# ramosian-glider/syzkaller

Measured on AMD Instinct MI355X. Metric: coverage PCs triaged/sec vs corpus signal (+ % HBM roofline), 1/2/4/8 MI355X, higher is better.
Workload: dtype u32

## Files before the change

syzkaller_amd/csrc/sg_bucket.hip:

```cpp
#include "sg_internal.h"

#include <algorithm>

#ifndef SG_EXP
#define SG_EXP 0
#endif


namespace sg {

#ifndef SG_HT_ABL
#define SG_HT_ABL 0
#endif
#ifndef SG_PT
#define SG_PT 16384
#endif
#ifndef SG_PTHREADS
#define SG_PTHREADS 1024
#endif
constexpr int kPT = SG_PT;
constexpr int kPThreads = SG_PTHREADS;
constexpr int kPWaves = kPThreads / 64;
constexpr int kPerWave = kPT / kPWaves;
constexpr int kSteps = kPerWave / 64;
// ... 725 lines not shown
  const uint64_t* goff;
};

__device__ __forceinline__ uint32_t shard_of(uint32_t s, uint32_t nshards) {
  s ^= s >> 16;
  s *= 0x85EBCA6Bu;
  s ^= s >> 13;
  s *= 0xC2B2AE35u;
  s ^= s >> 16;
  return (uint32_t)(((uint64_t)s * nshards) >> 32);
}

constexpr uint32_t kMaxShards = 64;

template <int kPer>
__device__ __forceinline__ void emit_pairs(const BucketArgs& a, const uint32_t (&sig)[kPer], const uint32_t (&rec)[kPer],
                                           uint32_t* shcnt) {
  constexpr uint32_t kNone = 0xFFFFFFFFu;
  __shared__ uint32_t ewc[16];
  __shared__ unsigned long long ebase;
  const int lane = threadIdx.x & 63, w = threadIdx.x >> 6, nw = blockDim.x >> 6;
  uint32_t c = 0;
#pragma unroll
  for (int k = 0; k < kPer; k++) c += rec[k] != kNone ? 1u : 0u;
  uint32_t incl = c;
#pragma unroll
  for (int o = 1; o < 64; o <<= 1) {
    const uint32_t y = __shfl_up(incl, o);
    if (lane >= o) incl += y;
  }
  if (lane == 63) ewc[w] = incl;
  __syncthreads();
  if (threadIdx.x == 0) {
    uint32_t acc = 0;
    for (int i = 0; i < nw; i++) {
      const uint32_t v = ewc[i];
      ewc[i] = acc;
      acc += v;
    }
    ebase = acc ? atomicAdd(a.npairs, (unsigned long long)acc) : 0ull;
  }
  __syncthreads();
  uint64_t pos = ebase + ewc[w] + incl - c;
#pragma unroll
  for (int k = 0; k < kPer; k++)
    if (rec[k] != kNone) {
      a.pairs[pos++] = make_uint2(sig[k], a.rec_base + rec[k]);
      if (a.shard_cnt) atomicAdd(&shcnt[shard_of(sig[k], a.nshards)], 1u);
    }
  __syncthreads();
}

template <int kPer>
__device__ __forceinline__ void emit_grouped(const BucketArgs& a, const uint32_t (&sig)[kPer], const uint32_t (&rec)[kPer],
                                             uint32_t* lcnt, unsigned long long* lbase) {
  constexpr uint32_t kNone = 0xFFFFFFFFu;
#pragma unroll
  for (int k = 0; k < kPer; k++)
    if (rec[k] != kNone) atomicAdd(&lcnt[rec[k] >> kGroupBits], 1u);
  __syncthreads();
  for (uint32_t g = threadIdx.x; g < a.NG; g += blockDim.x) {
    const uint32_t c = lcnt[g];
    lbase[g] = c ? a.goff[(uint64_t)g << kGroupBits] + atomicAdd(&a.gcur[g], (unsigned long long)c) : 0ull;
    lcnt[g] = 0;
  }
  __syncthreads();
#pragma unroll
  for (int k = 0; k < kPer; k++)
    if (rec[k] != kNone) {
      const uint32_t g = rec[k] >> kGroupBits;
      a.pairs[lbase[g] + atomicAdd(&lcnt[g], 1u)] = make_uint2(sig[k], rec[k]);
    }
  __syncthreads();
  for (uint32_t g = threadIdx.x; g < a.NG; g += blockDim.x) lcnt[g] = 0;
  __syncthreads();
}

__device__ __forceinline__ void flush_shard_counts(const BucketArgs& a, const uint32_t* shcnt) {
  if (a.shard_cnt)
    for (uint32_t i = threadIdx.x; i < a.nshards; i += blockDim.x)
      if (shcnt[i]) atomicAdd(&a.shard_cnt[i], (unsigned long long)shcnt[i]);
}

__global__ void k_bucket_compact(const uint4* __restrict__ bdesc, const uint32_t* __restrict__ lpos,
                                 uint32_t* __restrict__ blist_b, uint4* __restrict__ blist_q) {
  const uint32_t b = blockIdx.x * blockDim.x + threadIdx.x;
  if (b >= kNumBuckets) return;
  const uint4 q = bdesc[b];
  if (q.x < q.y) {
    blist_b[lpos[b]] = b;
    blist_q[lpos[b]] = q;
  }
}

__global__ void k_bucket_desc(const uint32_t* __restrict__ goff2, const uint32_t* __restrict__ gcount,
                              const uint32_t* __restrict__ cfirst, uint4* __restrict__ bdesc, uint32_t* __restrict__ nz) {
  const uint32_t b = blockIdx.x * blockDim.x + threadIdx.x;
  if (b >= kNumBuckets) return;
  const uint32_t d = b >> 8, f = b & 255, c0 = cfirst[d], nch = cfirst[d + 1] - c0;
  const uint32_t* row = goff2 + (uint64_t)f * *gcount + c0;
  const uint32_t lo = row[0], hi = row[nch];
  bdesc[b] = make_uint4(lo, hi, c0, nch);
  nz[b] = lo < hi ? 1u : 0u;
}

__global__ void k_bucket_groups(const uint32_t* __restrict__ goff2, const uint32_t* __restrict__ gcount,
                                const uint32_t* __restrict__ cbase, uint32_t NG, uint32_t* __restrict__ gbnd) {
  const uint64_t i = (uint64_t)blockIdx.x * blockDim.x + threadIdx.x;
  if (i >= (uint64_t)kNumBuckets * NG) return;
  const uint32_t b = (uint32_t)(i / NG), g = (uint32_t)(i % NG);
  gbnd[i] = goff2[(uint64_t)(b & 255) * *gcount + cbase[(b >> 8) * NG + g]];
}

__device__ __forceinline__ uint32_t group_of(const uint32_t* gb, uint32_t NG, uint32_t p) {
  uint32_t lo = 0, hi = NG;
  while (hi - lo > 1) {
    const uint32_t mid = (lo + hi) >> 1;
    if (gb[mid] <= p)
      lo = mid;
    else
      hi = mid;
  }
  return lo;
}

__device__ __forceinline__ uint32_t entry_record(uint32_t g, uint32_t x) { return (g << kGroupBits) | (x & 0xFFFFu); }

constexpr uint32_t kGroupWords = (kMaxGroups + kBThreads - 1) / kBThreads;
constexpr int kWPT = kBucketWords / kBThreads;
typedef uint32_t wvec __attribute__((ext_vector_type(kWPT)));
struct BucketPre {
  uint32_t msw[kBucketWords / kBThreads];
  uint32_t nsw[kBucketWords / kBThreads];
  uint32_t gw[kGroupWords];
};

__device__ __forceinline__ uint32_t round_pos(uint32_t base, int u) { return base + threadIdx.x * kBU + u; }

__device__ __forceinline__ void bucket_round_load(const BucketArgs& a, uint32_t base, uint32_t hi,
                                                  uint32_t (&x)[kBU]) {
  const uint4* p = reinterpret_cast<const uint4*>(a.in + base) + threadIdx.x * (kBU / 4);
#pragma unroll
  for (int j = 0; j < kBU / 4; j++) {
    uint4 v = make_uint4(0, 0, 0, 0);
    if (round_pos(base, 4 * j) < hi) {
      const v4u32 t = __builtin_nontemporal_load(reinterpret_cast<const v4u32*>(p + j));
      v = make_uint4(t[0], t[1], t[2], t[3]);
    }
    x[4 * j] = v.x;
    x[4 * j + 1] = v.y;
    x[4 * j + 2] = v.z;
    x[4 * j + 3] = v.w;
  }
}

__device__ __forceinline__ void bucket_pre_load(const BucketArgs& a, uint32_t b, BucketPre& P) {
  const uint64_t w0 = bucket_word(b, kWPT * threadIdx.x);
  wvec m = *reinterpret_cast<const wvec*>(a.mwords + w0);
  if (a.owords) m |= *reinterpret_cast<const wvec*>(a.owords + w0);
  wvec nw = {};
  if (a.nwords) nw = *reinterpret_cast<const wvec*>(a.nwords + w0);
#pragma unroll
  for (int j = 0; j < kWPT; j++) {
    P.msw[j] = m[j];
    P.nsw[j] = nw[j];
  }
  const uint32_t* gr = a.gbnd + (uint64_t)b * a.NG;
#pragma unroll
  for (int j = 0; j < (int)kGroupWords; j++) {
    const uint32_t i = j * kBThreads + threadIdx.x;
    P.gw[j] = i < a.NG ? gr[i] : 0u;
  }
}

__device__ __forceinline__ uint32_t list_bucket(const BucketArgs& a, uint32_t t, uint32_t nl, uint4* q) {
  if (t >= nl) return kNumBuckets;
  *q = a.blist_q[t];
  return a.blist_b[t];
}

#ifndef SG_LDS_BARRIER
#define SG_LDS_BARRIER 0
#endif
__device__ __forceinline__ void lds_barrier() {
#if SG_LDS_BARRIER
  asm volatile("s_waitcnt lgkmcnt(0)\n\ts_barrier" ::: "memory");
#else
  __syncthreads();
#endif
}

__device__ __forceinline__ uint32_t uni(uint32_t v) { return __builtin_amdgcn_readfirstlane(v); }
__device__ __forceinline__ uint4 uni(uint4 v) { return make_uint4(uni(v.x), uni(v.y), uni(v.z), uni(v.w)); }

constexpr uint32_t kMapMul = 0x6F4Bu;
constexpr uint32_t inv16(uint32_t c) {
  uint32_t x = c;
  for (int i = 0; i < 4; i++) x = (x * (2u - c * x)) & 0xFFFFu;
  return x;
}
constexpr uint32_t kMapInv = inv16(kMapMul);
static_assert(((kMapMul * kMapInv) & 0xFFFFu) == 1u, "kMapInv");
static_assert(kHash == 8192 && kMaxProbe <= 31, "13-bit slots, 5-bit displacements");
static_assert((uint64_t)kMaxGroups << kGroupBits <= (1u << 24), "records fit 24 bits");
constexpr uint32_t kRecMask = 0xFFFFFFu;

__device__ __forceinline__ uint32_t map_signal(uint32_t slot, uint32_t v) {
  const uint32_t home = (slot - ((v >> 24) & 31u)) & (kHash - 1);
  return (((home << 3) | (v >> 29)) * kMapInv) & 0xFFFFu;
}

__device__ __forceinline__ bool map_insert(uint32_t* ht, uint32_t sl, uint32_t rec, uint32_t disp0 = 0) {
  const uint32_t y = (sl * kMapMul) & 0xFFFFu;
  const uint32_t home = y >> 3, tag = y & 7u;
  for (uint32_t disp = disp0; disp < kMaxProbe; disp++) {
    const uint32_t mine = (tag << 29) | (disp << 24) | rec;
    uint32_t* slot = &ht[(home + disp) & (kHash - 1)];
    const uint32_t old = atomicCAS(slot, kEmpty, mine);
    if (old == kEmpty) return true;
    if ((old >> 24) == (mine >> 24)) {
      if ((old & kRecMask) > rec) atomicMin(slot, mine);
      return true;
    }
  }
  return false;
}

__device__ __forceinline__ uint32_t take_ticket(uint32_t* p) { return atomicAdd(p, 1u); }
__device__ __forceinline__ void take_wait(uint32_t&) {}

template <bool kDbg, int kEmit>
__global__ __launch_bounds__(kBThreads) __attribute__((amdgpu_waves_per_eu(kBWaves))) void k_bucket(BucketArgs a) {
  __shared__ uint32_t mslice[kBucketWords];
  __shared__ uint32_t nbits[kBucketWords];
  __shared__ uint32_t ht[kHash];
  __shared__ alignas(16) uint32_t gb[kMaxGroups];
  __shared__ uint32_t sh_fail;
  __shared__ uint32_t sh_b[2];
  __shared__ uint4 sh_q[2];
  __shared__ uint32_t shcnt[kEmit == 1 ? kMaxShards : 1];
  __shared__ uint32_t lcnt[kEmit == 2 ? kMaxGroups : 1];
  __shared__ unsigned long long lbase[kEmit == 2 ? kMaxGroups : 1];
  const int tid = threadIdx.x;
  if (kEmit == 1)
    for (uint32_t i = tid; i < kMaxShards; i += kBThreads) shcnt[i] = 0;
  if (kEmit == 2)
    for (uint32_t i = tid; i < kMaxGroups; i += kBThreads) lcnt[i] = 0;
  const uint32_t NG = a.NG;
  constexpr uint32_t kRound = kBThreads * kBU;
  const uint64_t t_start = kDbg ? wall_clock64() : 0;
  uint64_t n_buckets = 0, n_rounds = 0;
  uint64_t ph[7] = {0, 0, 0, 0, 0, 0, 0};
  uint64_t tk = kDbg ? clock64() : 0;
  for (uint32_t i = tid; i < kHash; i += kBThreads) ht[i] = kEmpty;
  for (uint32_t i = tid; i < kBucketWords; i += kBThreads) nbits[i] = 0;
  if (tid == 0) sh_fail = 0;
  const uint32_t nl = *a.nlist;
  uint32_t pend_t = 0;
  if (tid == 0) {
    uint4 q0 = make_uint4(0, 0, 0, 0), q1 = make_uint4(0, 0, 0, 0);
    sh_b[0] = list_bucket(a, blockIdx.x, nl, &q0);
    sh_q[0] = q0;
    sh_b[1] = list_bucket(a, gridDim.x + blockIdx.x, nl, &q1);
    sh_q[1] = q1;
    pend_t = take_ticket(a.ticket);
  }
  __syncthreads();
  uint32_t b = uni(sh_b[0]), b1 = uni(sh_b[1]);
  uint4 q = uni(sh_q[0]), q1 = uni(sh_q[1]);
  if (b >= kNumBuckets) {
    if (tid == 0) take_wait(pend_t);
    if (kDbg && tid == 0) {
      for (int j = 0; j < 8; j++) a.dbg[8 * blockIdx.x + j] = 0;
      a.dbg[8 * blockIdx.x] = t_start;
      a.dbg[8 * blockIdx.x + 1] = wall_clock64();
    }
    return;
  }
  uint32_t x[kBU], y[kBU];
  BucketPre P;
  bucket_round_load(a, q.x & ~3u, q.y, x);
  bucket_pre_load(a, b, P);
  while (b < kNumBuckets) {
    const uint32_t lo = q.x, hi = q.y;
    lds_barrier();
    {
      wvec mv;
#pragma unroll
      for (int j = 0; j < kWPT; j++) mv[j] = P.msw[j];
      reinterpret_cast<wvec*>(mslice)[tid] = mv;
    }
    uint32_t ns[kWPT];
#pragma unroll
    for (int j = 0; j < kWPT; j++) ns[j] = P.nsw[j];
#pragma unroll
    for (int j = 0; j < (int)kGroupWords; j++) {
      const uint32_t i = j * kBThreads + tid;
      if (i < kMaxGroups) gb[i] = i < NG ? P.gw[j] : kEmpty;
    }
    uint32_t pend_b = kNumBuckets;
    uint4 pend_q = make_uint4(0, 0, 0, 0);
    if (tid == 0) {
      take_wait(pend_t);
      pend_b = list_bucket(a, 2 * gridDim.x + pend_t, nl, &pend_q);
      pend_t = take_ticket(a.ticket);
      if (kEmit) take_wait(pend_t);
      sh_fail = 0;
    }
    lds_barrier();
    const uint32_t gbl = NG <= 64 ? gb[threadIdx.x & 63] : kEmpty;
    if (kDbg) {
      const uint64_t t = clock64();
      ph[0] += t - tk;
      tk = t;
    }
    n_buckets++;
    for (uint32_t base = lo & ~3u;;) {
      n_rounds++;
      const uint32_t next = base + kRound;
      const bool last = next >= hi;
      if (!last || b1 < kNumBuckets) bucket_round_load(a, last ? q1.x & ~3u : next, last ? q1.y : hi, y);
      if (last && b1 < kNumBuckets) bucket_pre_load(a, b1, P);
      const uint32_t p0 = round_pos(base, 0);
      const uint32_t failed = __hip_atomic_load(&sh_fail, __ATOMIC_RELAXED, __HIP_MEMORY_SCOPE_WORKGROUP);
      uint32_t mw[kBU];
#pragma unroll
      for (int u = 0; u < kBU; u++) mw[u] = mslice[x[u] >> 21];
      uint32_t cm = 0;
#pragma unroll
      for (int u = 0; u < kBU; u++) {
        const uint32_t i = p0 + u;
        const uint32_t miss = ((~mw[u]) >> ((x[u] >> 16) & 31)) & 1u;
        cm |= (miss & (i >= lo ? 1u : 0u) & (i < hi ? 1u : 0u)) << u;
      }
      if (kDbg) {
        asm volatile("s_waitcnt lgkmcnt(0)" ::: "memory");
        const uint64_t t = clock64();
        ph[4] += t - tk;
        tk = t;
      }
      uint32_t gu[kBU];
      if (NG <= 64) {
        const uint32_t pw = base + (threadIdx.x & ~63u) * kBU;
        const uint32_t nle = (uint32_t)__popcll(__ballot(gbl <= pw));
#pragma unroll
        for (int u = 0; u < kBU; u++) gu[u] = nle;
// ... 157 lines not shown
      }
      __syncthreads();
      uint64_t pos = ebase + ewc[w] + incl - c;
      if (c) {
#pragma unroll
        for (int k = 0; k < kOwn; k++) {
          const uint32_t i = k * kBThreads + tid;
          const uint32_t v = ht[i];
          if (v != kEmpty) {
            const uint32_t sl = map_signal(i, v);
            const uint32_t sg = part_sig((b << 16) | sl);
            a.pairs[pos++] = make_uint2(sg, a.rec_base + (v & kRecMask));
            if (a.shard_cnt) atomicAdd(&shcnt[shard_of(sg, a.nshards)], 1u);
            if (a.nwords || a.update) atomicOr(&nbits[sl >> 5], 1u << (sl & 31));
            ht[i] = kEmpty;
          }
        }
      }
      __syncthreads();
      if (a.update) {
        const wvec nb = reinterpret_cast<const wvec*>(nbits)[tid];
        const wvec mw = reinterpret_cast<const wvec*>(mslice)[tid];
        const uint64_t w0 = bucket_word(b, kWPT * tid);
#pragma unroll
        for (int j = 0; j < kWPT; j++)
          if (nb[j]) {
            a.mwords[w0 + j] = mw[j] | nb[j];
            if (a.nwords) a.nwords[w0 + j] = ns[j] | nb[j];
          }
      } else if (a.nwords) {
        const wvec nb = reinterpret_cast<const wvec*>(nbits)[tid];
        uint32_t* ng = a.nwords + bucket_word(b, kWPT * tid);
#pragma unroll
        for (int j = 0; j < kWPT; j++)
          if (nb[j]) ng[j] = ns[j] | nb[j];
      }
      reinterpret_cast<wvec*>(nbits)[tid] = wvec{};
    } else {
      constexpr int kOwn = kHash / kBThreads;
      {
#pragma unroll
        for (int k = 0; k < kOwn; k++) {
          const uint32_t i = k * kBThreads + tid;
          const uint32_t v = ht[i];
          ht[i] = kEmpty;
          if (v != kEmpty) {
            const uint32_t sl = map_signal(i, v);
            atomicOr(&nbits[sl >> 5], 1u << (sl & 31));
            a.rec_new[v & kRecMask] = 1;
          }
        }
        lds_barrier();
      }
      {
        const uint64_t w0 = bucket_word(b, kWPT * tid);
        uint32_t* mg = a.mwords + w0;
        uint32_t* ng = a.nwords ? a.nwords + w0 : nullptr;
        const wvec nb = reinterpret_cast<const wvec*>(nbits)[tid];
        uint32_t any = 0;
#pragma unroll
        for (int j = 0; j < kWPT; j++) any |= nb[j];
        if (any) {
          const wvec mw = reinterpret_cast<const wvec*>(mslice)[tid];
#pragma unroll
          for (int j = 0; j < kWPT; j++)
            if (nb[j]) {
              mg[j] = mw[j] | nb[j];
              if (ng) ng[j] = ns[j] | nb[j];
            }
          reinterpret_cast<wvec*>(nbits)[tid] = wvec{};
        }
      }
    }
    if (kDbg) {
      const uint64_t t = clock64();
      ph[3] += t - tk;
      tk = t;
    }
    lds_barrier();
    if (kDbg) {
      const uint64_t t = clock64();
      ph[6] += t - tk;
      tk = t;
    }
    b = b1;
    q = q1;
    b1 = uni(sh_b[0]);
    q1 = uni(sh_q[0]);
#pragma unroll
    for (int u = 0; u < kBU; u++) x[u] = y[u];
  }
  if (kEmit == 1) {
    __syncthreads();
    flush_shard_counts(a, shcnt);
  }
  if (kDbg && tid == 0) {
    a.dbg[8 * blockIdx.x] = t_start;
    a.dbg[8 * blockIdx.x + 1] = wall_clock64();
    a.dbg[8 * blockIdx.x + 2] = n_buckets;
    a.dbg[8 * blockIdx.x + 3] = n_rounds;
    for (int j = 0; j < 4; j++) a.dbg[8 * blockIdx.x + 4 + j] = ph[j];
    a.dbg[8 * gridDim.x + 3 * blockIdx.x] = ph[4];
    a.dbg[8 * gridDim.x + 3 * blockIdx.x + 1] = ph[5];
    a.dbg[8 * gridDim.x + 3 * blockIdx.x + 2] = ph[6];
  }
}

constexpr int kDThreads = 1024;
template <bool kEmit>
__global__ __launch_bounds__(kDThreads) void k_bucket_direct(BucketArgs a) {
  constexpr uint32_t kQ = 8192, kNQ = 65536 / kQ, kQW = kQ / 32;
  __shared__ uint32_t owner[kQ];
  __shared__ uint32_t mpart[kQW];
  __shared__ uint32_t nbits[kQW];
  __shared__ uint32_t gb[kMaxGroups];
  __shared__ uint32_t shcnt[kEmit ? kMaxShards : 1];
  __shared__ uint32_t lcnt[kEmit ? kMaxGroups : 1];
  __shared__ unsigned long long lbase[kEmit ? kMaxGroups : 1];
  const int tid = threadIdx.x;
  const uint32_t nsp = *a.nspill, NG = a.NG;
  if (kEmit) {
    for (uint32_t i = tid; i < kMaxShards; i += kDThreads) shcnt[i] = 0;
    for (uint32_t i = tid; i < kMaxGroups; i += kDThreads) lcnt[i] = 0;
    __syncthreads();
  }
  for (uint32_t job = blockIdx.x; job < nsp * kNQ; job += gridDim.x) {
    const uint32_t b = a.spill[job / kNQ], qq = job % kNQ;
    const uint4 q = a.bdesc[b];
    for (uint32_t i = tid; i < kQW; i += kDThreads) {
      const uint64_t w = bucket_word(b, qq * kQW + i);
      mpart[i] = a.mwords[w] | (a.owords ? a.owords[w] : 0u);
      nbits[i] = 0;
    }
    for (uint32_t i = tid; i < NG; i += kDThreads) gb[i] = a.gbnd[(uint64_t)b * NG + i];
    for (uint32_t i = tid; i < kQ; i += kDThreads) owner[i] = kEmpty;
    __syncthreads();
    for (uint32_t i = q.x + tid; i < q.y; i += kDThreads) {
      const uint32_t x = a.in[i];
      const uint32_t sl = x >> 16, sq = sl % kQ;
      if (sl / kQ != qq || ((mpart[sq >> 5] >> (sq & 31)) & 1u)) continue;
      atomicMin(&owner[sq], entry_record(group_of(gb, NG, i), x));
      atomicOr(&nbits[sq >> 5], 1u << (sq & 31));
    }
    __syncthreads();
    if (kEmit) {
      constexpr int kPer = kQ / kDThreads;
      uint32_t sig[kPer], rec[kPer];
#pragma unroll
      for (int k = 0; k < kPer; k++) {
        const uint32_t i = k * kDThreads + tid;
        sig[k] = part_sig((b << 16) | (qq * kQ + i));
        rec[k] = owner[i];
      }
      if (a.gcur)
        emit_grouped(a, sig, rec, lcnt, lbase);
      else
        emit_pairs(a, sig, rec, shcnt);
      for (uint32_t i = tid; i < kQW; i += kDThreads) {
        const uint32_t nb = nbits[i];
        if (!nb) continue;
        const uint64_t w = bucket_word(b, qq * kQW + i);
        if (a.update) a.mwords[w] = mpart[i] | nb;
        if (a.nwords) a.nwords[w] |= nb;
      }
    } else {
      for (uint32_t i = tid; i < kQ; i += kDThreads)
        if (owner[i] != kEmpty) a.rec_new[owner[i]] = 1;
      for (uint32_t i = tid; i < kQW; i += kDThreads) {
        const uint32_t nb = nbits[i];
        if (nb) {
          const uint64_t w = bucket_word(b, qq * kQW + i);
          a.mwords[w] = mpart[i] | nb;
          if (a.nwords) a.nwords[w] |= nb;
        }
      }
    }
    __syncthreads();
  }
  if (kEmit) flush_shard_counts(a, shcnt);
}

constexpr int kScanThreads = 1024;
constexpr int kScanPer = 16;
constexpr uint32_t kScanTile = kScanThreads * kScanPer;

__device__ __forceinline__ uint32_t block_excl_scan(uint32_t v, uint32_t* wsum, uint32_t* total) {
  const int tid = threadIdx.x, lane = tid & 63, w = tid >> 6;
// ... 52 lines not shown
  __shared__ uint32_t wsum[16];
  __shared__ uint32_t tot;
  uint32_t carry = 0;
  for (uint64_t b0 = 0; b0 < nb; b0 += kScanThreads) {
    const uint64_t i = b0 + threadIdx.x;
    const uint32_t v = i < nb ? sums[i] : 0u;
    const uint32_t ex = block_excl_scan(v, wsum, &tot);
    if (i < nb) sums[i] = carry + ex;
    carry += tot;
    __syncthreads();
  }
}

__global__ __launch_bounds__(kScanThreads) void k_scan32_apply(const uint32_t* __restrict__ in, uint64_t n,
                                                               const uint32_t* __restrict__ n_dev, uint32_t mul,
                                                               const uint32_t* __restrict__ sums,
                                                               uint32_t* __restrict__ out) {
  __shared__ uint32_t wsum[16];
  __shared__ uint32_t tot;
  n = scan_n(n, n_dev, mul);
  const uint64_t b_last = n ? (n - 1) / kScanTile : 0;
  if (blockIdx.x > b_last) return;
  const uint64_t base = (uint64_t)blockIdx.x * kScanTile + (uint64_t)threadIdx.x * kScanPer;
  const bool full = base + kScanPer <= n;
  uint32_t v[kScanPer];
  uint32_t s = 0;
  if (full) {
#pragma unroll
    for (int k = 0; k < kScanPer; k += 4) {
      const uint4 q = *reinterpret_cast<const uint4*>(in + base + k);
      v[k] = q.x;
      v[k + 1] = q.y;
      v[k + 2] = q.z;
      v[k + 3] = q.w;
    }
  } else {
#pragma unroll
    for (int k = 0; k < kScanPer; k++) v[k] = base + k < n ? in[base + k] : 0u;
  }
#pragma unroll
  for (int k = 0; k < kScanPer; k++) s += v[k];
  uint32_t run = (sums ? sums[blockIdx.x] : 0u) + block_excl_scan(s, wsum, &tot);
  uint32_t o[kScanPer];
#pragma unroll
  for (int k = 0; k < kScanPer; k++) {
    o[k] = run;
    run += v[k];
  }
  if (full) {
#pragma unroll
    for (int k = 0; k < kScanPer; k += 4)
      *reinterpret_cast<uint4*>(out + base + k) = make_uint4(o[k], o[k + 1], o[k + 2], o[k + 3]);
  } else {
#pragma unroll
    for (int k = 0; k < kScanPer; k++)
      if (base + k < n) out[base + k] = o[k];
  }
  if (blockIdx.x == b_last && threadIdx.x == kScanThreads - 1) out[n] = run;
}

static size_t scan32_ws(uint64_t n) { return (((n + kScanTile - 1) / kScanTile) * 4 + 255) & ~size_t(255); }

static int scan32(sg_ctx* ctx, const uint32_t* in, uint32_t* out, uint64_t n, uint32_t* scratch,
                  const uint32_t* n_dev = nullptr, uint32_t mul = 1) {
  ScopedTimer tm(ctx, "scan");
  const uint64_t nb = (n + kScanTile - 1) / kScanTile;
  if (nb == 0) {
    SG_HIP(hipMemsetAsync(out, 0, 4, ctx->stream));
    return SG_OK;
  }
  if (nb == 1) {
    hipLaunchKernelGGL(k_scan32_apply, dim3(1), dim3(kScanThreads), 0, ctx->stream, in, n, n_dev, mul,
                       (const uint32_t*)nullptr, out);
    SG_HIP(hipGetLastError());
    return SG_OK;
  }
  hipLaunchKernelGGL(k_scan32_reduce, dim3((uint32_t)nb), dim3(kScanThreads), 0, ctx->stream, in, n, n_dev, mul,
                     scratch);
  hipLaunchKernelGGL(k_scan32_top, dim3(1), dim3(kScanThreads), 0, ctx->stream, scratch, nb);
  hipLaunchKernelGGL(k_scan32_apply, dim3((uint32_t)nb), dim3(kScanThreads), 0, ctx->stream, in, n, n_dev, mul,
                     scratch, out);
  SG_HIP(hipGetLastError());
  return SG_OK;
}

constexpr uint32_t kFRemBits = 11;
constexpr uint32_t kFBuckets = 1u << (24 - kFRemBits);
constexpr uint32_t kFOvBlocks = 1984;
constexpr uint32_t kFPad = 0x8000u;
constexpr uint32_t kFSpill = 512;
constexpr uint32_t kFHMax = 4;
constexpr uint32_t kFIdx = 256 * kFHMax;
constexpr uint32_t kFSurvCap = 1u << 20;
constexpr uint32_t kFTableBits = 21;
constexpr int kFThreads = 1024;
#ifndef SG_FPARTS
#define SG_FPARTS 8
#endif
#ifndef SG_FU
#define SG_FU 4
#endif
#ifndef SG_FEH
#define SG_FEH 4
#endif
#ifndef SG_FABL
#define SG_FABL 0
#endif
constexpr uint32_t kFParts = SG_FPARTS;
constexpr uint32_t kFWgCap = 4 * kFSurvCap / (256 * kFParts);
constexpr unsigned long long kFEmpty = ~0ull;

struct M0F {
  uint4* tab;
  uint16_t* ovals;
  uint32_t* cursor;
  uint32_t* nspill;
  uint32_t* spill;
  uint32_t* nsurv;
  uint2* surv;
  uint32_t* wgcnt;
  unsigned long long* table;
};
static size_t m0f_bytes() {
  return (uint64_t)kFIdx * kFBuckets * 16 + (uint64_t)kFIdx * kFOvBlocks * 16 + kFIdx * 4 + 256 + kFIdx * 4 +
         (uint64_t)kFIdx * kFSpill * 4 + 256ull * kFParts * kFWgCap * 8 +
         256ull * kFParts * 4 + (8ull << kFTableBits);
}
static M0F m0f_bind(sg_ctx* ctx) {
  char* b = (char*)ctx->m0f;
  M0F f;
  f.tab = (uint4*)b;
  b += (uint64_t)kFIdx * kFBuckets * 16;
  f.ovals = (uint16_t*)b;
  b += (uint64_t)kFIdx * kFOvBlocks * 16;
  f.cursor = (uint32_t*)b;
  f.nsurv = f.cursor + kFIdx;
  f.nspill = f.cursor + kFIdx + 64;
  b += kFIdx * 4 + 256 + kFIdx * 4;
  f.spill = (uint32_t*)b;
  b += (uint64_t)kFIdx * kFSpill * 4;
  f.surv = (uint2*)b;
  b += 256ull * kFParts * kFWgCap * 8;
  f.wgcnt = (uint32_t*)b;
  b += 256ull * kFParts * 4;
  f.table = (unsigned long long*)b;
  return f;
}

template <int kLogH>
__global__ __launch_bounds__(256) void k_m0_index(const uint32_t* __restrict__ mwords, uint4* __restrict__ tab,
                                                   uint16_t* __restrict__ ovals, uint32_t* __restrict__ cursor,
                                                   uint32_t* __restrict__ nspill, uint32_t* __restrict__ spill,
                                                   uint32_t* __restrict__ flags) {
  constexpr int kQ = 16 >> kLogH;
  constexpr uint32_t kRB = kFRemBits - kLogH;
  const uint32_t dh = blockIdx.y, lane = threadIdx.x & 63;
  const uint32_t d = dh >> kLogH, h = dh & ((1u << kLogH) - 1);
  const uint32_t j = blockIdx.x * 256 + threadIdx.x;
  const uint4* src = reinterpret_cast<const uint4*>(mwords + ((uint64_t)d << 19) + ((uint64_t)h << (19 - kLogH)) +
                                                    (uint64_t)j * (4 * kQ));
  uint4 q[kQ];
#pragma unroll
  for (int i = 0; i < kQ; i++) q[i] = src[i];
  uint32_t n = 0;
#pragma unroll
  for (int i = 0; i < kQ; i++) n += __popc(q[i].x) + __popc(q[i].y) + __popc(q[i].z) + __popc(q[i].w);
// ... 401 lines not shown
  uint32_t* v2 = (uint32_t*)ws_at(ctx, bp.oV2);
    uint32_t* scr = (uint32_t*)ws_at(ctx, bp.oSC);
  const uint32_t T = (uint32_t)bp.T, G = (uint32_t)bp.gmax, NG = (uint32_t)bp.NG;
  const uint32_t* gcount = cbase + bp.ng;
  const bool dbg = ctx->debug_part;
  if (stages & 1) {
  Cuts c1{};
  c1.nA = bp.nA;
  c1.step = kPT;
  c1.nB = bp.nB;
  c1.n = n;
  c1.rec_off = d_off;
  c1.nrec = nrec;
  c1.start = tstart;
  c1.aux = trec;
  hipLaunchKernelGGL(k_cuts, dim3(div_up(bp.T + 1, 256)), dim3(256), 0, ctx->stream, c1);
  hipLaunchKernelGGL(k_group_tiles, dim3(div_up(bp.NG + 1, 256)), dim3(256), 0, ctx->stream, d_off, bp.nA, NG, T,
                     gt);
  {
    ScopedTimer tm(ctx, "p1_hist");
    if (trace)
      hipLaunchKernelGGL(k_hist_trace, dim3(T), dim3(kPThreads), 0, ctx->stream, d_vals, d_off, nrec,
                         (const uint32_t*)tstart, (const uint32_t*)trec, T, hist1, (uint64_t*)ws_at(ctx, bp.oKM));
    else if (((uintptr_t)d_vals & 15) == 0)
      hipLaunchKernelGGL(k_hist_rep<false>, dim3(T), dim3(kPThreads), 0, ctx->stream, d_vals,
                         (const uint32_t*)tstart, (const uint4*)nullptr, T, (const uint32_t*)nullptr, hist1);
    else
      hipLaunchKernelGGL(k_p1_hist, dim3(T), dim3(kPThreads), 0, ctx->stream, d_vals,
                         (const uint32_t*)tstart, hist1);
  }
  rc = scan32(ctx, hist1, goff1, 256 * bp.T, scr);
  if (rc) return rc;
  P1Args a1{d_vals, d_off, nrec, tstart, trec, T, goff1, hist1, v1, plane ? b1 : nullptr, nullptr,
            (const uint64_t*)ws_at(ctx, bp.oKM)};
  unsigned long long* p1dbg = nullptr;
  if (dbg) {
    SG_HIP(hipMalloc(&p1dbg, 64));
    SG_HIP(hipMemsetAsync(p1dbg, 0, 64, ctx->stream));
    a1.dbg = p1dbg;
  }
  {
    ScopedTimer tm(ctx, "p1_scatter");
    if (dbg && trace)
      hipLaunchKernelGGL((k_p1_scatter<true, true>), dim3(T), dim3(kPThreads), 0, ctx->stream, a1);
    else if (dbg)
      hipLaunchKernelGGL((k_p1_scatter<true, false>), dim3(T), dim3(kPThreads), 0, ctx->stream, a1);
    else if (trace)
      hipLaunchKernelGGL((k_p1_scatter<false, true>), dim3(T), dim3(kPThreads), 0, ctx->stream, a1);
    else
      hipLaunchKernelGGL((k_p1_scatter<false, false>), dim3(T), dim3(kPThreads), 0, ctx->stream, a1);
  }
  if (dbg) {
    unsigned long long h[8];
    SG_HIP(hipMemcpy(h, p1dbg, 64, hipMemcpyDeviceToHost));
    SG_HIP(hipFree(p1dbg));
    fprintf(stderr, "sg p1_scatter per tile (cycles, wave 0): load+meta %.0f build+lookup %.0f rank %.0f stage %.0f "
            "write %.0f (tiles %llu)\n", (double)h[0] / h[5], (double)h[1] / h[5], (double)h[2] / h[5],
            (double)h[3] / h[5], (double)h[4] / h[5], h[5]);
  }
  }
  if (!(stages & 2)) return SG_OK;
  hipLaunchKernelGGL(k_group_chunks, dim3(div_up(bp.ng, 256)), dim3(256), 0, ctx->stream, (const uint32_t*)goff1,
                     T, NG, (const uint32_t*)gt, bp.ng, nch);
  rc = scan32(ctx, nch, cbase, bp.ng, scr);
  if (rc) return rc;
  hipLaunchKernelGGL(k_chunk_list, dim3(div_up((bp.ng > bp.gmax ? bp.ng : bp.gmax) + 1, 256)), dim3(256), 0,
                     ctx->stream, (const uint32_t*)goff1, T, NG, (const uint32_t*)gt, bp.ng,
                     (const uint32_t*)cbase, bp.gmax, cstart, cgov, cfirst);
  hipLaunchKernelGGL(k_chunk_desc, dim3(div_up(bp.gmax, 256)), dim3(256), 0, ctx->stream, (const uint32_t*)cstart,
                     (const uint32_t*)cgov, gcount, bp.gmax, (const uint32_t*)goff1, T, NG, (const uint32_t*)gt,
                     cdesc, dtile);
  {
    ScopedTimer tm(ctx, "p2_hist");
    hipLaunchKernelGGL(k_hist_bytes, dim3(G), dim3(kHBThreads), 0, ctx->stream, (const uint8_t*)b1,
                       (const uint4*)cdesc, gcount, hist2);
  }
  rc = scan32(ctx, hist2, goff2, 256 * bp.gmax, scr, gcount, 256);
  if (rc) return rc;
  P2Args a2{v1, cdesc, dtile, gcount, goff1, trec, T, NG, goff2, hist2, v2};
  {
    ScopedTimer tm(ctx, "p2_scatter");
    hipLaunchKernelGGL(k_p2_scatter, dim3(G), dim3(kPThreads), 0, ctx->stream, a2);
  }
  uint32_t* bnz = (uint32_t*)ws_at(ctx, bp.oBN);
  uint32_t* blpos = (uint32_t*)ws_at(ctx, bp.oBP);
  hipLaunchKernelGGL(k_bucket_desc, dim3(kNumBuckets / 256), dim3(256), 0, ctx->stream, (const uint32_t*)goff2,
                     gcount, (const uint32_t*)cfirst, bdesc, bnz);
  hipLaunchKernelGGL(k_bucket_groups, dim3(div_up((uint64_t)kNumBuckets * NG, 256)), dim3(256), 0, ctx->stream,
                     (const uint32_t*)goff2, gcount, (const uint32_t*)cbase, NG, gbnd);
  rc = scan32(ctx, bnz, blpos, kNumBuckets, scr);
  if (rc) return rc;
  hipLaunchKernelGGL(k_bucket_compact, dim3(kNumBuckets / 256), dim3(256), 0, ctx->stream, (const uint4*)bdesc,
                     (const uint32_t*)blpos, (uint32_t*)ws_at(ctx, bp.oLB), (uint4*)ws_at(ctx, bp.oLQ));
  SG_HIP(hipGetLastError());
  return SG_OK;
}

static int buckets_one(sg_ctx* ctx, const BucketPlan& bp, uint32_t* mwords, uint32_t* nwords, uint8_t* d_rec_new,
                       const EmitArgs* emit, uint64_t n, uint64_t nrec, const uint32_t* owords = nullptr) {
  const uint32_t NG = (uint32_t)bp.NG;
  const uint32_t* cbase = (const uint32_t*)ws_at(ctx, bp.oCB);
  const uint32_t* gcount = cbase + bp.ng;
  uint4* bdesc = (uint4*)ws_at(ctx, bp.oBD);
  uint32_t* gbnd = (uint32_t*)ws_at(ctx, bp.oGB);
  uint32_t* v2 = (uint32_t*)ws_at(ctx, bp.oV2);
  uint32_t* nspill = (uint32_t*)ws_at(ctx, bp.oSP);
  uint32_t* blpos = (uint32_t*)ws_at(ctx, bp.oBP);
  const bool dbg = ctx->debug_part;
  BucketArgs ba{};
  ba.in = v2;
  ba.bdesc = bdesc;
  ba.gbnd = gbnd;
  ba.NG = NG;
  ba.mwords = mwords;
  ba.owords = owords;
  ba.nwords = nwords;
  ba.rec_new = d_rec_new;
  ba.nspill = nspill;
  ba.spill = nspill + 1;
  ba.ticket = (uint32_t*)ws_at(ctx, bp.oTK);
  if (emit) {
    ba.pairs = emit->pairs;
    ba.npairs = emit->npairs;
    ba.rec_base = emit->rec_base;
    ba.nshards = emit->nshards;
    ba.shard_cnt = emit->shard_cnt;
    ba.update = emit->update ? 1u : 0u;
    ba.gcur = emit->gcur;
    ba.goff = emit->goff;
  }
  uint32_t bgrid = persistent_grid(ctx, (const void*)k_bucket<false, 0>, kBThreads);
  const int64_t cap_blocks = ctx->opt[kOptBucketBlocks];
  if (cap_blocks > 0 && (uint64_t)cap_blocks < bgrid) bgrid = (uint32_t)cap_blocks;
  uint64_t* ddbg = nullptr;
  if (dbg) {
    SG_HIP(hipMalloc(&ddbg, (size_t)bgrid * 88));
    ba.dbg = ddbg;
  }
  SG_HIP(hipMemsetAsync(ba.ticket, 0, 4, ctx->stream));
  SG_HIP(hipMemsetAsync(nspill, 0, 4, ctx->stream));
  ba.blist_b = (const uint32_t*)ws_at(ctx, bp.oLB);
  ba.blist_q = (const uint4*)ws_at(ctx, bp.oLQ);
  ba.nlist = blpos + kNumBuckets;
  {
    ScopedTimer tm(ctx, "bucket_triage");
    if (emit && emit->gcur)
      hipLaunchKernelGGL((k_bucket<false, 2>), dim3(bgrid), dim3(kBThreads), 0, ctx->stream, ba);
    else if (emit)
      hipLaunchKernelGGL((k_bucket<false, 1>), dim3(bgrid), dim3(kBThreads), 0, ctx->stream, ba);
    else if (dbg)
      hipLaunchKernelGGL((k_bucket<true, 0>), dim3(bgrid), dim3(kBThreads), 0, ctx->stream, ba);
    else
      hipLaunchKernelGGL((k_bucket<false, 0>), dim3(bgrid), dim3(kBThreads), 0, ctx->stream, ba);
  }
  {
    ScopedTimer tm(ctx, "bucket_spill");
    if (emit)
      hipLaunchKernelGGL(k_bucket_direct<true>, dim3(512), dim3(kDThreads), 0, ctx->stream, ba);
    else
      hipLaunchKernelGGL(k_bucket_direct<false>, dim3(512), dim3(kDThreads), 0, ctx->stream, ba);
  }
  SG_HIP(hipGetLastError());
  if (dbg) {
    uint32_t g = 0, sp = 0;
    SG_HIP(hipMemcpyAsync(&g, gcount, 4, hipMemcpyDeviceToHost, ctx->stream));
    SG_HIP(hipMemcpyAsync(&sp, nspill, 4, hipMemcpyDeviceToHost, ctx->stream));
    SG_HIP(hipStreamSynchronize(ctx->stream));
    fprintf(stderr, "sg part: n=%llu nrec=%llu tiles=%llu chunks=%u (bound %llu) spilled_buckets=%u\n",
            (unsigned long long)n, (unsigned long long)nrec, (unsigned long long)bp.T, g,
            (unsigned long long)bp.gmax, sp);
    std::vector<uint4> bd(kNumBuckets);
    std::vector<uint64_t> hd((size_t)bgrid * 11);
    SG_HIP(hipMemcpy(bd.data(), bdesc, bd.size() * 16, hipMemcpyDeviceToHost));
    SG_HIP(hipMemcpy(hd.data(), ddbg, hd.size() * 8, hipMemcpyDeviceToHost));
    double qa = 0, qb = 0, qc = 0;
    for (uint32_t i = 0; i < bgrid; i++) {
      qa += hd[8 * bgrid + 3 * i];
      qb += hd[8 * bgrid + 3 * i + 1];
      qc += hd[8 * bgrid + 3 * i + 2];
    }
    SG_HIP(hipFree(ddbg));
    std::vector<uint32_t> sz(kNumBuckets);
    uint64_t rounds = 0;
    for (uint32_t b = 0; b < kNumBuckets; b++) {
      sz[b] = bd[b].y - bd[b].x;
      rounds += (sz[b] + 8191) / 8192;
    }
    std::sort(sz.begin(), sz.end());
    uint64_t t0 = ~0ull, t1 = 0;
    std::vector<double> dur;
    uint64_t maxr = 0;
    double phs[4] = {0, 0, 0, 0}, nbk = 0, nrd = 0;
    for (uint32_t i = 0; i < bgrid; i++) {
      t0 = std::min(t0, hd[8 * i]);
      t1 = std::max(t1, hd[8 * i + 1]);
      dur.push_back((hd[8 * i + 1] - hd[8 * i]) / 100.0);
      maxr = std::max(maxr, hd[8 * i + 3]);
      nbk += hd[8 * i + 2];
      nrd += hd[8 * i + 3];
      for (int j = 0; j < 4; j++) phs[j] += hd[8 * i + 4 + j];
    }
    fprintf(stderr, "sg bucket per bucket (cycles, wave 0): install %.0f | rounds: test %.0f insert %.0f tail %.0f | "
            "end barrier %.0f flush %.0f final barrier %.0f | rounds/bucket %.2f\n", phs[0] / nbk, qa / nbk, qb / nbk,
            phs[1] / nbk, phs[2] / nbk, phs[3] / nbk, qc / nbk, nrd / nbk);
    std::sort(dur.begin(), dur.end());
    fprintf(stderr,
            "sg bucket: sizes max=%u p99=%u median=%u rounds=%llu | blocks=%u span=%.1fus dur min=%.1f med=%.1f "
            "max=%.1f us, max rounds/block=%llu\n",
            sz.back(), sz[kNumBuckets * 99 / 100], sz[kNumBuckets / 2], (unsigned long long)rounds, bgrid,
            (t1 - t0) / 100.0, dur.front(), dur[dur.size() / 2], dur.back(), (unsigned long long)maxr);
  }
  return SG_OK;
}

static int m0_filter(sg_ctx* ctx, const BucketPlan& bp, uint32_t* mwords, uint32_t* nwords, uint8_t* d_rec_new,
                     bool* done) {
  *done = false;
  if (!ctx->m0f) {
    SG_HIP(hipMalloc(&ctx->m0f, m0f_bytes()));
    const M0F f0 = m0f_bind(ctx);
    SG_HIP(hipMemsetAsync(f0.table, 0xFF, 8ull << kFTableBits, ctx->stream));
  }
  const M0F f = m0f_bind(ctx);
  const uint32_t T = (uint32_t)bp.T;
  SG_HIP(hipMemsetAsync(f.cursor, 0, kFIdx * 4 + 256 + kFIdx * 4, ctx->stream));
  const int logh = ctx->opt[kOptM0Halves] >= 0 ? (int)ctx->opt[kOptM0Halves] : ctx->m0f_logh;
  {
    ScopedTimer tm(ctx, "m0_index");
    const dim3 ig(kFBuckets / 256, 256u << logh);
    if (logh == 0)
      hipLaunchKernelGGL(k_m0_index<0>, ig, dim3(256), 0, ctx->stream, (const uint32_t*)mwords, f.tab, f.ovals,
                         f.cursor, f.nspill, f.spill, f.nsurv);
    else if (logh == 1)
      hipLaunchKernelGGL(k_m0_index<1>, ig, dim3(256), 0, ctx->stream, (const uint32_t*)mwords, f.tab, f.ovals,
                         f.cursor, f.nspill, f.spill, f.nsurv);
    else
      hipLaunchKernelGGL(k_m0_index<2>, ig, dim3(256), 0, ctx->stream, (const uint32_t*)mwords, f.tab, f.ovals,
                         f.cursor, f.nspill, f.spill, f.nsurv);
  }
  {
    ScopedTimer tm(ctx, "m0_filter");
    auto kf = logh == 0 ? k_m0_filter<0> : logh == 1 ? k_m0_filter<1> : k_m0_filter<2>;
    hipLaunchKernelGGL(kf, dim3(kFParts >> logh, 256, 1u << logh), dim3(kFThreads), 0, ctx->stream,
                       (const uint32_t*)ws_at(ctx, bp.oV1), (const uint32_t*)ws_at(ctx, bp.oO1), T,
                       (const uint4*)f.tab, (const uint16_t*)f.ovals, (const uint32_t*)f.cursor,
                       (const uint32_t*)f.nspill, (const uint32_t*)f.spill, f.surv, f.nsurv, f.wgcnt);
  }
  SG_HIP(hipGetLastError());
  uint32_t nsv[3] = {0, 0, 0};
  SG_HIP(hipMemcpyAsync(nsv, f.nsurv, 12, hipMemcpyDeviceToHost, ctx->stream));
  SG_HIP(hipStreamSynchronize(ctx->stream));
  const uint32_t ns = nsv[0];
  ctx->m0f_survivors = nsv[1] ? kFSurvCap + 1 : ns;
  if (nsv[1] || ns > kFSurvCap) {
    ctx->m0f_fallback++;
    ctx->m0f_last = 0;
    if (ctx->opt[kOptM0Halves] < 0 && nsv[2] && ctx->m0f_logh < 1) {
      ctx->m0f_logh++;
    } else if (ctx->opt[kOptM0Filter] < 0) {
      ctx->m0f_backoff = ctx->m0f_backoff ? std::min<uint32_t>(2 * ctx->m0f_backoff, 64) : 1;
      ctx->m0f_skip = ctx->m0f_backoff;
    }
    return SG_OK;
  }
  if (ns) {
    ScopedTimer tm(ctx, "m0_tail");
    hipLaunchKernelGGL(k_m0_tail_insert, dim3(4, 256 * kFParts), dim3(256), 0, ctx->stream,
                       (const uint2*)f.surv, (const uint32_t*)f.wgcnt,
                       (const uint32_t*)ws_at(ctx, bp.oV1), (const uint32_t*)ws_at(ctx, bp.oO1), T,
                       (const uint32_t*)ws_at(ctx, bp.oTR), (const uint32_t*)mwords, f.table);
    hipLaunchKernelGGL(k_m0_tail_flush, dim3((1u << kFTableBits) / 256), dim3(256), 0, ctx->stream, f.table, mwords,
                       nwords, d_rec_new);
  }
  SG_HIP(hipGetLastError());
  ctx->m0f_used++;
  ctx->m0f_last = 1;
  ctx->m0f_backoff = ctx->m0f_skip = 0;
  *done = true;
  return SG_OK;
}

__global__ void k_top_plane(const uint32_t* __restrict__ v1, uint64_t n, uint8_t* __restrict__ b1) {
  for (uint64_t i = ((uint64_t)blockIdx.x * blockDim.x + threadIdx.x) * 4; i < n;
       i += (uint64_t)gridDim.x * blockDim.x * 4) {
    if (i + 4 <= n && ((uintptr_t)(v1 + i) & 15) == 0) {
      const uint4 q = *reinterpret_cast<const uint4*>(v1 + i);
      *reinterpret_cast<uint32_t*>(b1 + i) = (q.x >> 24) | ((q.y >> 24) << 8) | ((q.z >> 24) << 16) | (q.w & 0xFF000000u);
    } else {
      for (uint64_t k = i; k < i + 4 && k < n; k++) b1[k] = (uint8_t)(v1[k] >> 24);
    }
  }
}

// ... 593 lines not shown
```

Before: 131.4 billion.

## Order bucket work list by descending size class for load balance

Replaces the nonzero-flag scan with a per-block histogram of bucket size classes (log-scale, 4 sub-bins per octave). A single-block order kernel scans these counts so the compacted list puts the largest buckets first, and compaction ranks each bucket within its class. Each block's second initial bucket now comes from the mirrored index, which pairs large and small buckets. The goal is to shrink the tail where a few large buckets finish last in the dynamically ticketed bucket kernel. It adds some shared-memory ranking work and debug timing for the first bucket.

```diff
diff --git a/syzkaller_amd/csrc/sg_bucket.hip b/syzkaller_amd/csrc/sg_bucket.hip
--- a/syzkaller_amd/csrc/sg_bucket.hip
+++ b/syzkaller_amd/csrc/sg_bucket.hip
@@ -831,26 +831,58 @@
       if (shcnt[i]) atomicAdd(&a.shard_cnt[i], (unsigned long long)shcnt[i]);
 }
 
-__global__ void k_bucket_compact(const uint4* __restrict__ bdesc, const uint32_t* __restrict__ lpos,
-                                 uint32_t* __restrict__ blist_b, uint4* __restrict__ blist_q) {
-  const uint32_t b = blockIdx.x * blockDim.x + threadIdx.x;
-  if (b >= kNumBuckets) return;
+constexpr int kListT = 256;
+constexpr uint32_t kListBlocks = kNumBuckets / kListT;
+constexpr uint32_t kSizeClasses = 128;
+constexpr uint32_t kListCounts = (kSizeClasses - 1) * kListBlocks;
+static_assert(kNumBuckets % kListT == 0 && kListCounts <= kNumBuckets, "the counts fit the list-position array");
+
+__device__ __forceinline__ uint32_t size_class(uint32_t n) {
+  if (n < 4) return n;
+  const uint32_t k = 31u - (uint32_t)__builtin_clz(n);
+  return 4 * k + ((n >> (k - 2)) & 3u);
+}
+
+__device__ __forceinline__ uint32_t list_count_at(uint32_t c, uint32_t blk) {
+  return (kSizeClasses - 1 - c) * kListBlocks + blk;
+}
+
+__global__ __launch_bounds__(kListT) void k_bucket_compact(const uint4* __restrict__ bdesc,
+                                                            const uint32_t* __restrict__ lbase,
+                                                            uint32_t* __restrict__ blist_b, uint4* __restrict__ blist_q) {
+  __shared__ alignas(16) uint32_t cls[kListT];
+  const uint32_t tid = threadIdx.x, b = blockIdx.x * kListT + tid;
   const uint4 q = bdesc[b];
-  if (q.x < q.y) {
-    blist_b[lpos[b]] = b;
-    blist_q[lpos[b]] = q;
-  }
-}
-
-__global__ void k_bucket_desc(const uint32_t* __restrict__ goff2, const uint32_t* __restrict__ gcount,
-                              const uint32_t* __restrict__ cfirst, uint4* __restrict__ bdesc, uint32_t* __restrict__ nz) {
-  const uint32_t b = blockIdx.x * blockDim.x + threadIdx.x;
-  if (b >= kNumBuckets) return;
+  const uint32_t c = q.x < q.y ? size_class(q.y - q.x) : 0u;
+  cls[tid] = c;
+  __syncthreads();
+  if (c == 0) return;
+  uint32_t rank = 0;
+  for (uint32_t j = 0; j < (uint32_t)kListT; j += 4) {
+    const uint4 k = *reinterpret_cast<const uint4*>(&cls[j]);
+    rank += (k.x == c && j < tid ? 1u : 0u) + (k.y == c && j + 1 < tid ? 1u : 0u) + (k.z == c && j + 2 < tid ? 1u : 0u) +
+            (k.w == c && j + 3 < tid ? 1u : 0u);
+  }
+  const uint32_t pos = lbase[list_count_at(c, blockIdx.x)] + rank;
+  blist_b[pos] = b;
+  blist_q[pos] = q;
+}
+
+__global__ __launch_bounds__(kListT) void k_bucket_desc(const uint32_t* __restrict__ goff2,
+                                                         const uint32_t* __restrict__ gcount,
+                                                         const uint32_t* __restrict__ cfirst, uint4* __restrict__ bdesc,
+                                                         uint32_t* __restrict__ lcount) {
+  __shared__ uint32_t cnt[kSizeClasses];
+  const uint32_t tid = threadIdx.x, b = blockIdx.x * kListT + tid;
+  if (tid < kSizeClasses) cnt[tid] = 0;
+  __syncthreads();
   const uint32_t d = b >> 8, f = b & 255, c0 = cfirst[d], nch = cfirst[d + 1] - c0;
   const uint32_t* row = goff2 + (uint64_t)f * *gcount + c0;
   const uint32_t lo = row[0], hi = row[nch];
   bdesc[b] = make_uint4(lo, hi, c0, nch);
-  nz[b] = lo < hi ? 1u : 0u;
+  if (lo < hi) atomicAdd(&cnt[size_class(hi - lo)], 1u);
+  __syncthreads();
+  if (tid >= 1 && tid < kSizeClasses) lcount[list_count_at(tid, blockIdx.x)] = cnt[tid];
 }
 
 __global__ void k_bucket_groups(const uint32_t* __restrict__ goff2, const uint32_t* __restrict__ gcount,
@@ -998,7 +1030,7 @@
   const uint32_t NG = a.NG;
   constexpr uint32_t kRound = kBThreads * kBU;
   const uint64_t t_start = kDbg ? wall_clock64() : 0;
-  uint64_t n_buckets = 0, n_rounds = 0;
+  uint64_t n_buckets = 0, n_rounds = 0, t_first = 0;
   uint64_t ph[7] = {0, 0, 0, 0, 0, 0, 0};
   uint64_t tk = kDbg ? clock64() : 0;
   for (uint32_t i = tid; i < kHash; i += kBThreads) ht[i] = kEmpty;
@@ -1010,7 +1042,7 @@
     uint4 q0 = make_uint4(0, 0, 0, 0), q1 = make_uint4(0, 0, 0, 0);
     sh_b[0] = list_bucket(a, blockIdx.x, nl, &q0);
     sh_q[0] = q0;
-    sh_b[1] = list_bucket(a, gridDim.x + blockIdx.x, nl, &q1);
+    sh_b[1] = list_bucket(a, 2 * gridDim.x - 1 - blockIdx.x, nl, &q1);
     sh_q[1] = q1;
     pend_t = take_ticket(a.ticket);
   }
@@ -1334,6 +1366,7 @@
       const uint64_t t = clock64();
       ph[6] += t - tk;
       tk = t;
+      if (n_buckets == 1) t_first = wall_clock64();
     }
     b = b1;
     q = q1;
@@ -1355,6 +1388,7 @@
     a.dbg[8 * gridDim.x + 3 * blockIdx.x] = ph[4];
     a.dbg[8 * gridDim.x + 3 * blockIdx.x + 1] = ph[5];
     a.dbg[8 * gridDim.x + 3 * blockIdx.x + 2] = ph[6];
+    a.dbg[11 * gridDim.x + blockIdx.x] = t_first;
   }
 }
 
@@ -1573,6 +1607,48 @@
                      scratch, out);
   SG_HIP(hipGetLastError());
   return SG_OK;
+}
+
+constexpr int kOrderRows = (kSizeClasses - 1 + 3) / 4;
+static_assert(kListBlocks == 256 && kScanThreads == 4 * 256 && kSizeClasses - 1 <= 128, "k_bucket_order's geometry");
+__global__ __launch_bounds__(kScanThreads) void k_bucket_order(uint32_t* __restrict__ lcount,
+                                                                uint32_t* __restrict__ nlist) {
+  __shared__ alignas(16) uint32_t wtot[kSizeClasses][4];
+  __shared__ uint32_t rowbase[kSizeClasses];
+  const uint32_t tid = threadIdx.x, grp = tid >> 8, tg = tid & 255, wv = tg >> 6, lane = tid & 63;
+  uint32_t v[kOrderRows], ex[kOrderRows];
+#pragma unroll
+  for (int r = 0; r < kOrderRows; r++) {
+    const uint32_t row = grp + 4 * r;
+    v[r] = row < kSizeClasses - 1 ? lcount[row * kListBlocks + tg] : 0u;
+  }
+#pragma unroll
+  for (int r = 0; r < kOrderRows; r++) {
+    const uint32_t incl = sgd::wave_incl_add(v[r]);
+    ex[r] = incl - v[r];
+    if (lane == 63) wtot[grp + 4 * r][wv] = incl;
+  }
+  __syncthreads();
+#pragma unroll
+  for (int r = 0; r < kOrderRows; r++) {
+    const uint4 w = *reinterpret_cast<const uint4*>(wtot[grp + 4 * r]);
+    ex[r] += (wv > 0 ? w.x : 0u) + (wv > 1 ? w.y : 0u) + (wv > 2 ? w.z : 0u);
+    if (tg == 255) rowbase[grp + 4 * r] = ex[r] + v[r];
+  }
+  __syncthreads();
+  if (tid < 64) {
+    const uint32_t a = rowbase[2 * tid], b = rowbase[2 * tid + 1];
+    const uint32_t incl = sgd::wave_incl_add(a + b);
+    rowbase[2 * tid] = incl - a - b;
+    rowbase[2 * tid + 1] = incl - b;
+    if (tid == 63) *nlist = incl;
+  }
+  __syncthreads();
+#pragma unroll
+  for (int r = 0; r < kOrderRows; r++) {
+    const uint32_t row = grp + 4 * r;
+    if (row < kSizeClasses - 1) lcount[row * kListBlocks + tg] = rowbase[row] + ex[r];
+  }
 }
 
 constexpr uint32_t kFRemBits = 11;
@@ -2140,15 +2216,16 @@
     ScopedTimer tm(ctx, "p2_scatter");
     hipLaunchKernelGGL(k_p2_scatter, dim3(G), dim3(kPThreads), 0, ctx->stream, a2);
   }
-  uint32_t* bnz = (uint32_t*)ws_at(ctx, bp.oBN);
   uint32_t* blpos = (uint32_t*)ws_at(ctx, bp.oBP);
-  hipLaunchKernelGGL(k_bucket_desc, dim3(kNumBuckets / 256), dim3(256), 0, ctx->stream, (const uint32_t*)goff2,
-                     gcount, (const uint32_t*)cfirst, bdesc, bnz);
+  hipLaunchKernelGGL(k_bucket_desc, dim3(kListBlocks), dim3(kListT), 0, ctx->stream, (const uint32_t*)goff2, gcount,
+                     (const uint32_t*)cfirst, bdesc, blpos);
   hipLaunchKernelGGL(k_bucket_groups, dim3(div_up((uint64_t)kNumBuckets * NG, 256)), dim3(256), 0, ctx->stream,
                      (const uint32_t*)goff2, gcount, (const uint32_t*)cbase, NG, gbnd);
-  rc = scan32(ctx, bnz, blpos, kNumBuckets, scr);
-  if (rc) return rc;
-  hipLaunchKernelGGL(k_bucket_compact, dim3(kNumBuckets / 256), dim3(256), 0, ctx->stream, (const uint4*)bdesc,
+  {
+    ScopedTimer tm(ctx, "scan");
+    hipLaunchKernelGGL(k_bucket_order, dim3(1), dim3(kScanThreads), 0, ctx->stream, blpos, blpos + kNumBuckets);
+  }
+  hipLaunchKernelGGL(k_bucket_compact, dim3(kListBlocks), dim3(kListT), 0, ctx->stream, (const uint4*)bdesc,
                      (const uint32_t*)blpos, (uint32_t*)ws_at(ctx, bp.oLB), (uint4*)ws_at(ctx, bp.oLQ));
   SG_HIP(hipGetLastError());
   return SG_OK;
@@ -2192,7 +2269,7 @@
   if (cap_blocks > 0 && (uint64_t)cap_blocks < bgrid) bgrid = (uint32_t)cap_blocks;
   uint64_t* ddbg = nullptr;
   if (dbg) {
-    SG_HIP(hipMalloc(&ddbg, (size_t)bgrid * 88));
+    SG_HIP(hipMalloc(&ddbg, (size_t)bgrid * 96));
     ba.dbg = ddbg;
   }
   SG_HIP(hipMemsetAsync(ba.ticket, 0, 4, ctx->stream));
@@ -2228,7 +2305,7 @@
             (unsigned long long)n, (unsigned long long)nrec, (unsigned long long)bp.T, g,
             (unsigned long long)bp.gmax, sp);
     std::vector<uint4> bd(kNumBuckets);
-    std::vector<uint64_t> hd((size_t)bgrid * 11);
+    std::vector<uint64_t> hd((size_t)bgrid * 12);
     SG_HIP(hipMemcpy(bd.data(), bdesc, bd.size() * 16, hipMemcpyDeviceToHost));
     SG_HIP(hipMemcpy(hd.data(), ddbg, hd.size() * 8, hipMemcpyDeviceToHost));
     double qa = 0, qb = 0, qc = 0;
@@ -2267,6 +2344,10 @@
             "max=%.1f us, max rounds/block=%llu\n",
             sz.back(), sz[kNumBuckets * 99 / 100], sz[kNumBuckets / 2], (unsigned long long)rounds, bgrid,
             (t1 - t0) / 100.0, dur.front(), dur[dur.size() / 2], dur.back(), (unsigned long long)maxr);
+    if (hd[2])
+      fprintf(stderr, "sg bucket: block 0: first bucket %.1f us, %llu buckets, %llu rounds, ends %.1f us into the span\n",
+              (hd[11 * (size_t)bgrid] - hd[0]) / 100.0, (unsigned long long)hd[2], (unsigned long long)hd[3],
+              (hd[1] - t0) / 100.0);
   }
   return SG_OK;
 }
```

Result: no change. 132.8 billion, median of 6 (+1.1%).
